# sithu/ByzantineRandomizedConsensus

Hardware: AMD Instinct MI355X
Metric: decided consensus instances/sec (node) at n=64,f=21 (higher is better)
Workload: dtype u32

## Files before the change

byzantinerandomizedconsensus_amd/csrc/brc_step.h:

```cpp
#pragma once
#include "brc_internal.h"
#include "schedule.h"

namespace brc {

constexpr uint32_t NOKEY = 0xFFFFFFFFu;
constexpr uint32_t TB_S = 1, TB_E = 2, TB_R = 4, TB_SH = 12, TB_KEY = (1u << TB_SH) - 1u;
constexpr uint32_t KL_SND_SH = 15, KL_DT_SH = 21, KL_RESTR = 1u << 25;

template <int NPAD> struct MaskOf { using type = uint64_t; };
template <> struct MaskOf<4> { using type = uint8_t; };
template <> struct MaskOf<8> { using type = uint8_t; };
template <> struct MaskOf<16> { using type = uint16_t; };
template <> struct MaskOf<32> { using type = uint32_t; };

template <typename T> __device__ __forceinline__ uint32_t popc(T x) { return (uint32_t)__popcll((uint64_t)x); }


__device__ __forceinline__ uint32_t dpp_row_or(uint32_t x) {
    x |= (uint32_t)__builtin_amdgcn_mov_dpp((int)x, 0xB1, 0xF, 0xF, true);
    x |= (uint32_t)__builtin_amdgcn_mov_dpp((int)x, 0x4E, 0xF, 0xF, true);
    x |= (uint32_t)__builtin_amdgcn_mov_dpp((int)x, 0x141, 0xF, 0xF, true);
    x |= (uint32_t)__builtin_amdgcn_mov_dpp((int)x, 0x140, 0xF, 0xF, true);
    return x;
// ... 66 lines not shown
        x = (x | (x >> 3)) & 0x0303030303030303ull; x = (x | (x >> 6)) & 0x000F000F000F000Full;
        x = (x | (x >> 12)) & 0x000000FF000000FFull;
        return (x | (x >> 24)) & 0xFFFFull;
    }
    if (G == 8) {
        x = (x | (x >> 7)) & 0x0003000300030003ull; x = (x | (x >> 14)) & 0x0000000F0000000Full;
        return (x | (x >> 28)) & 0xFFull;
    }
    if (G == 16) {
        x = (x | (x >> 15)) & 0x0000000300000003ull;
        return (x | (x >> 30)) & 0xFull;
    }
    return (x | (x >> 31)) & 0x3ull;
}

template <int I> struct IC { static constexpr int value = I; };
template <int N> struct Unrolled {
    template <typename F> __device__ __forceinline__ static void run(F&& f) {
        Unrolled<N - 1>::run(f);
        f(IC<N - 1>{});
    }
};
template <> struct Unrolled<0> {
    template <typename F> __device__ __forceinline__ static void run(F&&) {}
};

__device__ __forceinline__ uint32_t uni32(uint32_t x) { return (uint32_t)__builtin_amdgcn_readfirstlane((int)x); }
__device__ __forceinline__ uint64_t uni64(uint64_t x) {
    return (uint64_t)uni32((uint32_t)x) | ((uint64_t)uni32((uint32_t)(x >> 32)) << 32);
}
__device__ __forceinline__ uint64_t readlane64(uint64_t x, int l) {
    return (uint64_t)(uint32_t)__builtin_amdgcn_readlane((int)(uint32_t)x, l) |
           ((uint64_t)(uint32_t)__builtin_amdgcn_readlane((int)(uint32_t)(x >> 32), l) << 32);
}

template <typename T> using gptr_t = __attribute__((address_space(1))) T*;
template <typename T> __device__ __forceinline__ gptr_t<T> gp(T* p) { return (gptr_t<T>)p; }

__device__ __forceinline__ InjDev load_inj(const InjDev* p) {
    const gptr_t<const uint64_t> q = gp((const uint64_t*)p);
    const uint64_t w[3] = {q[0], q[1], q[2]};
    InjDev r;
    __builtin_memcpy(&r, w, 24);
    r.dst_hi[0] = r.dst_hi[1] = r.dst_hi[2] = 0;
    return r;
}

__device__ __forceinline__ uint32_t m_s1(uint64_t m) { return (uint32_t)(m & 0xFFFF); }
__device__ __forceinline__ uint32_t m_tsend(uint64_t m) { return (uint32_t)((m >> 16) & 0xFFFF); }
__device__ __forceinline__ uint32_t m_tquiet(uint64_t m) { return (uint32_t)((m >> 32) & 0xFFFF); }
__device__ __forceinline__ uint32_t m_sender(uint64_t m) { return (uint32_t)((m >> 48) & 0xFF); }
__device__ __forceinline__ uint32_t m_value(uint64_t m) { return (uint32_t)((m >> 56) & 0x7F); }
constexpr uint64_t M_RESTRICTED = 1ull << 63;
__device__ __forceinline__ uint64_t m_pack(uint32_t s1, uint32_t tsend, uint32_t tquiet, uint32_t sender, uint32_t value) {
    return (uint64_t)(s1 & 0xFFFF) | ((uint64_t)(tsend & 0xFFFF) << 16) | ((uint64_t)(tquiet & 0xFFFF) << 32) |
           ((uint64_t)(sender & 0xFF) << 48) | ((uint64_t)(value & 0xFF) << 56);
}
__device__ __forceinline__ uint64_t m_with_tquiet(uint64_t m, uint32_t q) {
    return (m & ~(0xFFFFull << 32)) | ((uint64_t)(q & 0xFFFF) << 32);
}

__device__ __forceinline__ void brb_cell_update(uint32_t& fl, uint32_t& ec, uint32_t& rc, bool s_arr,
                                                uint32_t ea, uint32_t ra, uint32_t T_echo, uint32_t T_amp,
                                                uint32_t T_del, bool& echo_send, bool& ready_send, bool& deliver) {
    const bool open = !(fl & F_DEL);
    const bool es_st = open && s_arr && !(fl & F_EEX);
    echo_send = es_st && !(fl & F_ES);
    fl |= es_st ? (F_EEX | F_ES) : 0u;
    const bool e_on = open && ea != 0;
    const uint32_t checked = (fl & F_EEX) ? ea : ea - 1u;
    fl |= e_on ? F_EEX : 0u;
    ec += e_on ? ea : 0u;
    const bool r1s = e_on && checked != 0 && ec >= T_echo && !(fl & F_REX);
    const bool r1 = r1s && !(fl & F_RS);
    fl |= r1s ? (F_REX | F_RS) : 0u;
    const bool r_on = open && ra != 0;
    const bool rex = (fl & F_REX) != 0;
    const uint32_t lo = rex ? rc + 1u : 2u, hi = rex ? rc + ra : ra;
    fl |= r_on ? F_REX : 0u;
    rc += r_on ? ra : 0u;
    const bool any = r_on && hi >= lo;
    const uint32_t alo = max(lo, T_amp), ahi = min(hi, T_del - 1u);
    const bool r2 = any & !(fl & F_EEX) & (alo <= ahi) & !(fl & F_RS);
    fl |= r2 ? F_RS : 0u;
    deliver = any && hi >= T_del;
    fl |= deliver ? F_DEL : 0u;
    ready_send = r1 || r2;
}

__device__ __forceinline__ void brb_cell_update_spec(uint32_t& fl, uint32_t& ec, uint32_t& rc, bool s_arr,
                                                     uint32_t ea, uint32_t ra, uint32_t T_echo, uint32_t T_amp,
                                                     uint32_t T_del, bool& echo_send, bool& ready_send, bool& deliver) {
    const bool open = !(fl & F_DEL);
    echo_send = open && s_arr && !(fl & F_ES);
    fl |= echo_send ? F_ES : 0u;
    ec += open ? ea : 0u;
    rc += open ? ra : 0u;
    ready_send = open && !(fl & F_RS) && (ec >= T_echo || rc >= T_amp);
    fl |= ready_send ? F_RS : 0u;
    deliver = open && rc >= T_del;
    fl |= deliver ? F_DEL : 0u;
}

__device__ __forceinline__ void brb_cell_update_beb(uint32_t& fl, bool s_arr, bool& echo_send, bool& ready_send,
                                                    bool& deliver) {
    deliver = s_arr && !(fl & F_DEL);
// ... 34 lines not shown
    const uint64_t w = r.lo ^ ((r.lo ^ r.hi) & (0ull - (uint64_t)((s >> 3) & 1u)));
    return (uint32_t)(w >> (8u * (s & 7u))) & 0xFFu;
}
__device__ __forceinline__ Ring16 ring_put(Ring16 r, uint32_t tl, uint32_t t, uint32_t c) {
    if (tl == NEVER || t - tl >= 16u) {
        r.lo = r.hi = 0;
    } else {
        for (uint32_t s = tl + 1u; s != t + 1u; ++s) {
            const uint64_t m = ~(0xFFull << (8u * (s & 7u)));
            if (s & 8u) r.hi &= m; else r.lo &= m;
        }
    }
    const uint64_t v = (uint64_t)min(c, RING_MAX) << (8u * (t & 7u)), m = ~(0xFFull << (8u * (t & 7u)));
    if (t & 8u) r.hi = (r.hi & m) | v; else r.lo = (r.lo & m) | v;
    return r;
}

#ifndef BRC_NL_MSTORE
#define BRC_NL_MSTORE 1
#endif
#ifndef BRC_LPK
#define BRC_LPK 1
#endif
#ifndef BRC_MIN_WAVES
#define BRC_MIN_WAVES 4
#endif
#ifndef BRC_MIN_WAVES_LEAN
#define BRC_MIN_WAVES_LEAN 4
#endif
#ifndef BRC_MIN_WAVES_LEAN_SPEC
#define BRC_MIN_WAVES_LEAN_SPEC 4
#endif
#ifndef BRC_SPEC_MULTI
#define BRC_SPEC_MULTI 1
#endif
#ifndef BRC_PERKEY_CNT
#define BRC_PERKEY_CNT 1
#endif
#ifndef BRC_BRANCHLESS
#define BRC_BRANCHLESS 0
#endif
#ifndef BRC_NOEARLY
#define BRC_NOEARLY 0
#endif
#ifndef BRC_LCHUNK_SPEC
#define BRC_LCHUNK_SPEC 4
#endif
#ifndef BRC_DACC
#define BRC_DACC 1
#endif
#ifndef BRC_OOBST
#define BRC_OOBST 1
#endif
#ifndef BRC_PK
#define BRC_PK 1
#endif
constexpr int TCLS = BRC_TYPED_ER ? 5 : 4;
constexpr int tcls_tb(int c) { return c == 1 ? 2 : c == 2 ? 4 : c == 3 ? 1 : c == 4 ? 6 : -1; }

typedef uint16_t u16x2 __attribute__((ext_vector_type(2)));
__device__ __forceinline__ uint32_t pk_add(uint32_t a, uint32_t b) {
    return __builtin_bit_cast(uint32_t, __builtin_bit_cast(u16x2, a) + __builtin_bit_cast(u16x2, b));
}
__device__ __forceinline__ uint32_t pk_sub(uint32_t a, uint32_t b) {
    return __builtin_bit_cast(uint32_t, __builtin_bit_cast(u16x2, a) - __builtin_bit_cast(u16x2, b));
}
__device__ __forceinline__ uint32_t pk_min(uint32_t a, uint32_t b) {
    return __builtin_bit_cast(uint32_t, __builtin_elementwise_min(__builtin_bit_cast(u16x2, a), __builtin_bit_cast(u16x2, b)));
}
__device__ __forceinline__ uint32_t pk_max(uint32_t a, uint32_t b) {
    return __builtin_bit_cast(uint32_t, __builtin_elementwise_max(__builtin_bit_cast(u16x2, a), __builtin_bit_cast(u16x2, b)));
}
__device__ __forceinline__ uint32_t pk_ge(uint32_t a, uint32_t b) { return (~pk_sub(a, b) >> 15) & 0x10001u; }
__device__ __forceinline__ uint32_t pk2(uint32_t x) { return x | (x << 16); }

#ifdef BRC_STAMPS
#define BRC_NSTAMPS 24
__device__ unsigned long long brc_stamps[BRC_NSTAMPS];
#endif
template <int NPAD, int MODE> constexpr bool lean_kernel() { return NPAD == 64 && MODE != KMODE_CONN && MODE != KMODE_XREF; }

#ifndef BRC_MIN_WAVES_EV
#define BRC_MIN_WAVES_EV 2
#endif
template <int NPAD, int DM, bool EV, int MODE, int NLR>
__global__ __launch_bounds__(64 * WPB, (EV ? BRC_MIN_WAVES_EV
                                           : lean_kernel<NPAD, MODE>() ? (MODE == BRC_MODE_SPEC ? BRC_MIN_WAVES_LEAN_SPEC
                                                                                              : BRC_MIN_WAVES_LEAN)
                                                                       : BRC_MIN_WAVES))
void brc_step(const Params* __restrict__ pp) {
    const Params& P = *pp;
    constexpr bool SPEC = MODE == BRC_MODE_SPEC, BEB = MODE == BRC_MODE_BEB, CONN = MODE == KMODE_CONN;
    constexpr bool LEAN = lean_kernel<NPAD, MODE>();
    constexpr bool TYPED = typed_list(LEAN, EV, MODE);
    static_assert(NLR == 0 || (LEAN && NLR == 2), "register delay masks: lean kernels, two delays");
    constexpr uint32_t CW = CONN ? 5 : 1;
    using T = typename MaskOf<NPAD>::type;
    constexpr uint32_t RS = ring_steps(DM);
    constexpr int IPW = 64 / NPAD;
    constexpr uint32_t AT = act_types(LEAN, IPW);
    constexpr bool PSEG = BRC_PSEG && !LEAN && IPW > 1;
    constexpr uint32_t NVAL = value_ids(!LEAN), VB = LEAN ? 2u : 3u, VMASK = NVAL - 1u;
    constexpr uint32_t VREP = LEAN ? 0x55u : 0x249249u;
    extern __shared__ __attribute__((aligned(16))) uint64_t smem[];

    const int wid = (int)uni32(threadIdx.x / 64), lane = threadIdx.x % 64;
    const uint64_t item = (uint64_t)blockIdx.x * WPB + wid;
    if (item >= P.nitems) return;
    const uint32_t n = P.n, NK = P.NK, Q = P.Q, NV = P.NV, D = P.D, nkw = P.nkw;
    const uint32_t T_echo = P.T_echo, T_amp = P.T_amp, T_del = P.T_del;
    const uint32_t qsh = (uint32_t)__ffs(Q) - 1u, Qm = Q - 1u, ksh = qsh + (uint32_t)__ffs(NV) - 1u;
    const uint32_t nL = NLR ? 0u : P.nL;
    const uint32_t h_words = cons_words(SPEC, (uint32_t)sizeof(T), Q, NV, NVAL);
    const bool seen_on = NV > 1;
    const uint32_t l_words = (nL * 64 * (uint32_t)sizeof(T) + 7) / 8;
    uint64_t* s_meta = smem + (size_t)wid * (lds_bytes_per_wave(NPAD, NK, nkw, nL, SPEC, Q, NV, RS, LEAN, TYPED) / 8);
    uint64_t* s_act = s_meta + IPW * NK;
    constexpr bool DBG = LEAN && SPEC;
    const uint32_t dbw = DBG ? 0u : 64u * nkw;
    uint64_t* s_dbits = s_act + RS * nkw * AT;
    T* s_hm = (T*)(s_dbits + dbw);
    T* s_seen = s_hm;
    uint32_t* s_cnt = (uint32_t*)(s_seen + (seen_on ? Q * 64 : 0u));
    T* s_L = (T*)(s_dbits + dbw + h_words);
    uint16_t* s_gen = (uint16_t*)(s_dbits + dbw + h_words + l_words);
    uint16_t* s_klist = s_gen + (LEAN ? 0u : ((IPW * NK + 3) & ~3u));
    const uint32_t KLS = NK + 2 * KPAD;
    constexpr bool KL32 = LEAN && (!SPEC || BRC_KL32_SPEC);
    uint32_t* s_klist32 = (uint32_t*)s_klist;
    uint64_t* s_injc = (uint64_t*)(s_klist + ((KLS * (PSEG ? IPW : 1u) + 3) & ~3u));

    const int seg = lane / NPAD, d = lane % NPAD, segbase = seg * NPAD;
    const uint64_t inst = item * IPW + seg;
    const bool iex = inst < P.instances;
    const uint64_t g = P.inst_offset + inst;
    const uint64_t all64 = (n >= 64) ? ~0ull : ((1ull << n) - 1);
    const T allm = (T)all64;
    const uint64_t segbits = (NPAD == 64) ? ~0ull : (((1ull << NPAD) - 1) << segbase);
    const uint32_t mbase = seg * NK;

    ItemState its = P.items[item];
    uint32_t t = LEAN ? uni32(its.t) : its.t, inj_pos = LEAN ? uni32(its.inj_pos) : its.inj_pos;
    uint32_t ep = LEAN ? uni32(its.epoch) : 0u;
    const uint32_t inj_off = gp(P.inj_off)[item], inj_cnt = gp(P.inj_cnt)[item];
    uint32_t injc_base = 0x80000000u;
    auto inj_at = [&](uint32_t pos) -> InjDev {
        if constexpr (LEAN) {
// ... 86 lines not shown
    const uint32_t maxout = hibit(outset);
    const uint32_t dset = wave_or_all(outset);
    uint64_t dlist = 0;
    uint32_t ndl = 0;
    for (uint32_t ds = dset; ds; ds &= ds - 1) dlist |= (uint64_t)(__ffs(ds) - 1) << (4 * ndl++);
    dlist = uni64(dlist); ndl = uni32(ndl);
    T RL0 = 0, RL1 = 0;
    constexpr bool LPK = NLR == 0 && BRC_LPK && sizeof(T) * DM <= 8;
    uint64_t Lpk = 0;
    uint32_t dly0 = 0, dly1 = 0;
    uint64_t OV0 = 0, OV1 = 0;
    if constexpr (NLR != 0) {
        if (ndl > 2) ovf = true;
        dly0 = ndl > 0 ? (uint32_t)(dlist & 15) + 1u : 0u;
        dly1 = ndl > 1 ? (uint32_t)((dlist >> 4) & 15) + 1u : 0u;
#pragma unroll
        for (int i = 0; i < DM; ++i) {
            if ((uint32_t)i + 1 == dly0) RL0 = L[i];
            if ((uint32_t)i + 1 == dly1) RL1 = L[i];
        }
        if (ndl > 0) OV0 = uni64(readlane64(outv, (int)dly0 - 1));
        if (ndl > 1) OV1 = uni64(readlane64(outv, (int)dly1 - 1));
    } else {
        uint32_t j = 0;
#pragma unroll
        for (int i = 0; i < DM; ++i)
            if ((dset >> i) & 1) {
                if (j < nL) s_L[j * 64 + lane] = L[i];
                if constexpr (LPK) Lpk |= (uint64_t)L[i] << ((j * 8 * sizeof(T)) & 63);
                ++j;
            }
        if (j > nL) ovf = true;
    }
    const uint64_t mk_ov = (lane & 1) ? OV1 : OV0;
    auto Lmask = [&](uint32_t j) -> T {
        if constexpr (NLR != 0) return j == 0 ? RL0 : RL1;
        else if constexpr (LPK) return (T)(Lpk >> ((j * 8 * sizeof(T)) & 63));
        else return s_L[j * 64 + lane];
    };
    const gptr_t<uint64_t> mycells = gp(P.cells) + item * (uint64_t)(NK + 1) * CW * 64 + lane;
    const gptr_t<uint64_t> gdbits = gp(P.dbits) + item * (uint64_t)nkw * 64 + lane;
    const __amdgpu_buffer_rsrc_t crs =
        __builtin_amdgcn_make_buffer_rsrc((void*)((uint32_t*)P.cells + item * (uint64_t)(NK + 1) * 64), (short)0,
                                          (int)((NK + 1) * 256u), 0x00020000);
    const uint32_t lv4 = (uint32_t)lane * 4u;
    auto cld = [&](uint32_t k) -> uint32_t { return __builtin_amdgcn_raw_buffer_load_b32(crs, lv4, k * 256u, 0); };
    auto cst = [&](uint32_t k, uint32_t v) { __builtin_amdgcn_raw_buffer_store_b32(v, crs, lv4, k * 256u, 0); };
    auto cst_if = [&](uint32_t k, uint32_t v, bool wr) {
        if constexpr (BRC_OOBST) __builtin_amdgcn_raw_buffer_store_b32(v, crs, wr ? lv4 : 0x80000000u, k * 256u, 0);
        else if (wr) cst(k, v);
    };
    uint32_t clr = 0;
    auto flush_clears = [&]() {
        if constexpr (LEAN) {
            for (uint64_t b = __ballot(clr != 0); b; b &= b - 1) {
                const int L = __ffsll((unsigned long long)b) - 1;
                for (uint32_t cm = uni32((uint32_t)__builtin_amdgcn_readlane((int)clr, L)); cm; cm &= cm - 1) {
                    const uint32_t k = ((uint32_t)L * NV) * Q + (uint32_t)__ffs(cm) - 1u;
                    cst(k, C32_FRESH);
                }
            }
            clr = 0;
        }
    };
    auto rebase = [&]() {
        if constexpr (LEAN) {
            const uint32_t nep = t - C32_KEEP, delta = nep - ep;
            for (uint32_t k = 0; k < NK; ++k) {
                if (m_s1(uni64(s_meta[k])) == 0) continue;
                const uint32_t c = cld(k);
                uint32_t oE = (c >> C32_OE_SH) & 127u, oR = c >> C32_OR_SH;
                if (oE < C32_OLD) oE = oE >= delta ? oE - delta : C32_OLD;
                if (oR < C32_OLD) oR = oR >= delta ? oR - delta : C32_OLD;
                cst(k, (c & ((1u << C32_OE_SH) - 1u)) | (oE << C32_OE_SH) | (oR << C32_OR_SH));
            }
            ep = nep;
        }
    };

    uint64_t c0 = 0, c1 = 0;
    const size_t li = item * 64 + lane;
    const bool cons_lane = honest && P.protocol == BRC_PROTO_CONSENSUS;
    if (cons_lane) { c0 = gp(P.cons0)[li]; c1 = gp(P.cons1)[li]; }
    if constexpr (SPEC) {
        const T* gseen = (const T*)P.hmask;
        const uint32_t* gcnt = (const uint32_t*)((const char*)P.hmask + (seen_on ? P.nitems * Q * 64 * sizeof(T) : 0));
        for (uint32_t q = 0; q < Q; ++q) {
            if (seen_on) s_seen[q * 64 + lane] = cons_lane ? gp(gseen)[(item * Q + q) * 64 + lane] : (T)0;
            s_cnt[q * 64 + lane] = cons_lane ? gp(gcnt)[(item * Q + q) * 64 + lane] : 0u;
        }
    } else {
        for (uint32_t v = 0; v < NVAL; ++v)
            s_hm[v * 64 + lane] = cons_lane ? gp((const T*)P.hmask)[(item * NVAL + v) * 64 + lane] : (T)0;
    }
    uint32_t round = c0 & 0xFFFF, phase = (c0 >> 16) & 0xF, nvals = (c0 >> 20) & 0xF;
    uint32_t order = (c0 >> 24) & 0xFFFFFF, vcount = (c0 >> 48) & 0xFFFF;
    uint32_t dcount = c1 & 0xFFFF, frnd = (c1 >> 16) & 0xFFFF, ft = (c1 >> 32) & 0xFFFF;
    uint32_t fval = (c1 >> 48) & 0xFF, lval = (c1 >> 56) & 0xFF;

    uint32_t xs_n = LEAN ? 0u : uni32(gp(P.xsn)[item]);
    auto xs_ld = [&](uint32_t i) -> uint64_t { return uni64(gp(P.xsend)[item * (uint64_t)(3 * XSEND_MAX) + i]); };

    uint32_t st_msgs = 0, st_arr = 0, st_cells = 0, st_del = 0, st_loads = 0, st_smax = 0;
    uint32_t st_bcast = 0;
    uint32_t nk_lean = 0, nk_skip = 0;

    auto log_ev = [&](uint32_t kind, uint32_t node, uint32_t type, uint32_t a, uint32_t b, uint32_t v) {
        if (EV) {
            const unsigned long long i = atomicAdd(P.event_count, 1ull);
            if (i < P.event_cap) {
                brc_event e;
                e.instance = inst; e.t = t; e.kind = (uint8_t)kind; e.node = (uint8_t)node;
                e.type = (uint8_t)type; e.value = (uint8_t)v; e.a = a; e.b = b;
                P.events[i] = e;
            }
        }
    };
    auto mark_lane = [&](uint32_t k, uint32_t ds, uint32_t ty) {
        while (ds) {
            const uint32_t i = __ffs(ds) - 1; ds &= ds - 1;
            const uint32_t row = (t + i + 1) & (RS - 1);
            if (!LEAN || ty != BRC_SEND)
                atomicOr((unsigned long long*)&s_act[(row * AT + (LEAN ? ty - BRC_ECHO : PSEG ? (uint32_t)seg : 0u)) * nkw + (k >> 6)],
                         1ull << (k & 63));
            lane_rows |= 1u << row;
        }
    };
    auto ring_busy = [&](uint32_t k) -> bool {
        const uint32_t kw = k >> 6, cur = t & (RS - 1);
        uint64_t acc = 0;
#pragma unroll 1
        for (uint32_t r = 0; r < RS; ++r)
            if (r != cur) acc |= s_act[(r * AT + 0) * nkw + kw] | s_act[(r * AT + 1) * nkw + kw];
        return (acc >> (k & 63)) & 1ull;
    };
    auto send_key_now = [&](uint32_t s, uint32_t v) {
        const uint32_t k = (d * NV) * Q + (s & Qm);
        const uint64_t m = s_meta[mbase + k];
        if ((m_s1(m) != 0 && (t < m_tquiet(m) || (LEAN && ring_busy(k)))) || s >= P.s_limit) { ovf = true; return; }
        if (!LEAN) s_gen[mbase + k] = (uint16_t)(((s_gen[mbase + k] & GEN_MASK) + 1) & GEN_MASK);
        if (LEAN) clr |= 1u << (s & Qm);
        s_meta[mbase + k] = m_pack(s + 1, t, t + maxout, d, v);
        mark_lane(k, outset, BRC_SEND);
        q_until = max(q_until, t + maxout);
        st_msgs += n;
        st_smax = max(st_smax, s);
        log_ev(BRC_EV_SEND, d, BRC_SEND, d * NV, s, v);
    };
    bool defer_sends = false;
    uint32_t sq_s = 0, sq_n = 0;
    SendQ<VB> sq_v;
    sq_v.clear();
    auto send_key = [&](uint32_t s, uint32_t v) {
        if (defer_sends) {
            if (sq_n == 0) sq_s = s;
            if (s == sq_s + sq_n && sq_n < SENDQ_MAX) { sq_v.put(sq_n, v & VMASK); ++sq_n; }
            else ovf = true;
            return;
        }
        send_key_now(s, v);
    };
    auto flush_sends = [&]() {
        for (uint32_t i = 0; i < sq_n; ++i) send_key_now(sq_s + i, sq_v.get(i) & VMASK);
        sq_n = 0; sq_v.clear();
    };
    auto get_max_val = [&](uint32_t bound2) -> uint32_t {
        for (uint32_t i = 0; i < nvals; ++i) {
            const uint32_t v = (order >> (VB * i)) & VMASK;
            if (2 * popc(s_hm[v * 64 + lane]) > bound2) return v;
        }
        return 0;
    };
    auto cons_reset = [&]() {
        vcount = 0; nvals = 0; order = 0;
        for (uint32_t v = 0; v < NVAL; ++v) s_hm[v * 64 + lane] = 0;
    };
    auto cons_after = [&]() {
        if (vcount >= P.T_cnt && phase == 1) {
            const uint32_t prop = get_max_val(P.bound_p1);
            phase = 2; cons_reset();
            send_key(2 * (round - 1) + 1, prop);
        }
        if (vcount >= P.T_cnt && phase == 2) {
            const uint32_t dec = get_max_val(P.bound_p2);
            ++dcount;
            if (dcount == 1) { frnd = round; ft = t; fval = dec; }
            lval = dec;
            log_ev(BRC_EV_DECIDE, d, 0, round, dec, dec);
            ++round; phase = 1; cons_reset();
            send_key(2 * (round - 1), dec);
        }
    };
    auto cons_deliver_vh = [&](uint32_t v, uint32_t host) {
        const uint32_t x = order ^ (v * VREP);
        const uint32_t valid = (1u << (VB * nvals)) - 1u;
// ... 83 lines not shown
                if (c > RING_MAX) {
                    badinj = true;
                } else {
                    sent = true;
                    ring = ring_put(ring, tl, t, c);
                    mycells[ri] = ring.lo;
                    mycells[ri + 64] = ring.hi;
                    log_ev((wv & bit) ? BRC_EV_COPY : BRC_EV_SEND, d, r.type, (k >> qsh), r.s, m_value(m));
                    wv = ((wv | bit) & ~(0xFFFFull << sh)) | ((uint64_t)t << sh);
                    mycells[(size_t)k * (CW * 64)] = wv;
                    st_msgs += n;
                }
            } else if (!(wv & bit)) {
                sent = true;
                wv |= bit;
                wv = (wv & ~(0xFFFFull << sh)) | ((uint64_t)t << sh);
                mycells[(size_t)k * (CW * 64)] = wv;
                st_msgs += n;
                log_ev(BRC_EV_SEND, d, r.type, (k >> qsh), r.s, m_value(m));
            }
        }
        return sent;
    };
    auto msg_marks = [&](const InjDev& r, bool mine, bool sent) {
        const uint32_t k = r.slot;
        const uint32_t os = wave_or(sent ? outset : 0u);
        if (os) {
            if (lane == 0) mark_lane(k, os, r.type);
            const uint32_t myq = seg_max<NPAD>(sent ? t + maxout : 0u);
            if (mine && myq) {
                if (d == 0) {
                    const uint64_t m = s_meta[mbase + k];
                    if (myq > m_tquiet(m)) s_meta[mbase + k] = m_with_tquiet(m, myq);
                }
                q_until = max(q_until, myq);
            }
        }
    };

    auto send_rec = [&](const InjDev& r, const uint32_t os) -> bool {
        const bool is_send = r.kind == BRC_INJ_SEND;
        const uint32_t k = r.slot;
        bool fresh = false;
        if (d == 0) {
            uint64_t m = s_meta[mbase + k];
            uint32_t gen = LEAN ? 0u : s_gen[mbase + k] & GEN_MASK;
            const bool declared = m_s1(m) == r.s + 1u && m_tsend(m) == NEVER && is_send;
            if ((!declared && m_s1(m) != 0 && (t < m_tquiet(m) || (LEAN && ring_busy(k)))) || r.s >= P.s_limit) {
                ovf = true;
            } else {
                uint32_t tq = m_tquiet(m);
                if (!declared) { gen = (gen + 1) & GEN_MASK; tq = t + 1; fresh = true; }
                if (is_send) tq = max(tq, t + hibit(os));
                m = m_pack(r.s + 1, is_send ? t : NEVER, tq, r.node, (uint32_t)(uint8_t)r.value);
                s_meta[mbase + k] = m;
                const bool restricted = is_send && (r.dst & all64) != all64;
                if (!LEAN) s_gen[mbase + k] = (uint16_t)(gen | (restricted ? GEN16_RESTRICTED : 0u));
                if (LEAN && restricted) s_meta[mbase + k] = m | M_RESTRICTED;
                st_smax = max(st_smax, (uint32_t)r.s);
                if (is_send) {
                    gp(P.kdst)[inst * NK + k] = r.dst;
                    mark_lane(k, os, BRC_SEND);
                    st_msgs += __popcll(r.dst & all64);
                    log_ev(BRC_EV_SEND, r.node, BRC_SEND, (k >> qsh), r.s, (uint32_t)(uint8_t)r.value);
                }
            }
        }
        return fresh;
    };
    auto send_delay_set = [&](const InjDev& r, const bool mine) -> uint32_t {
        uint32_t myset = 0;
        if (r.kind == BRC_INJ_SEND && mine && honest && ((r.dst >> d) & 1ull)) {
            uint32_t j = 0;
            for (uint32_t ds = dset; ds; ds &= ds - 1, ++j)
                if ((Lmask(j) >> r.node) & 1) myset = 1u << (__ffs(ds) - 1);
        }
        return myset;
    };

    auto do_actions = [&]() -> bool {
        bool mine_any = false;
        const bool running = status == BRC_RUNNING;
        if (its.initialized == 0 && t == 0) {
            if (P.protocol == BRC_PROTO_CONSENSUS && P.proposals != BRC_PROPOSALS_NONE && honest && running) {
                const uint32_t v = (P.proposals == BRC_PROPOSALS_PHILOX) ? proposal_id(P.seed, g, d)
                                                                         : (uint32_t)gp(P.prop)[inst * n + d];
                round = 1; phase = 1;
                send_key(0, v & (SPEC ? 3u : VMASK));
                if constexpr (SPEC) spec_advance();
            }
            flush_clears();
        }
        while (inj_pos < inj_cnt) {
            const InjDev r = inj_at(inj_pos);
            if (r.t != t) break;
            ++inj_pos;
            const bool mine = running && seg == (int)r.seg;
            mine_any |= mine;
            if (r.kind == BRC_INJ_PROPOSE) {
                if (mine && honest && d == r.node) {
                    round = 1; phase = 1; send_key(0, (uint32_t)r.value & (SPEC ? 3u : VMASK));
                    if constexpr (SPEC) spec_advance();
                }
            } else if (r.kind == BRC_INJ_DELIVER) {
                if constexpr (!SPEC) {
                    if (mine && honest && d == r.node) cons_deliver_vh((uint32_t)r.value & VMASK, r.slot);
                }
            } else if (!LEAN && IPW > 1 && (r.kind == BRC_INJ_SEND || r.kind == BRC_INJ_KEY) && !(r.type & 2u)) {
                const uint32_t p0 = inj_pos - 1;
                uint32_t p1 = inj_pos;
                while (p1 < inj_cnt && p1 - injc_base < INJ_CACHE) {
                    const InjDev q = inj_at(p1);
                    if (q.t != t || (q.kind != BRC_INJ_SEND && q.kind != BRC_INJ_KEY) || (q.type & 2u)) break;
                    ++p1;
                }
                inj_pos = p1;
                uint32_t myrecs = 0;
                for (uint32_t p = p0; p < p1; ++p)
                    if (seg == (int)inj_at(p).seg) myrecs |= 1u << (p - p0);
                while (__any(myrecs != 0)) {
                    InjDev q = r;
                    const bool has = myrecs != 0;
                    if (has) {
                        const uint32_t i = (uint32_t)__ffs(myrecs) - 1u;
                        myrecs &= myrecs - 1;
                        q = inj_at(p0 + i);
                    }
                    const bool mq = has && running;
                    mine_any |= mq;
                    const uint32_t os = seg_or<NPAD, uint32_t>(send_delay_set(q, mq));
                    if (mq) {
                        send_rec(q, os);
                        q_until = max(q_until, t + hibit(os));
                    }
                }
            } else if (r.kind == BRC_INJ_SEND || r.kind == BRC_INJ_KEY) {
                const uint32_t os = wave_or(send_delay_set(r, mine));
                if (!LEAN && (r.type & 2u)) {
                    if (mine && d == 0) {
                        const uint32_t k = r.slot;
                        const uint64_t m = s_meta[mbase + k];
                        if (m_s1(m) != r.s + 1u || m_tsend(m) == NEVER) {
                            badinj = true;
                        } else {
                            if (t + hibit(os) > m_tquiet(m)) s_meta[mbase + k] = m_with_tquiet(m, t + hibit(os));
                            mark_lane(k, os, BRC_SEND);
                            st_msgs += __popcll(r.dst & all64);
                            if (!(r.type & 1u)) log_ev(BRC_EV_SEND, r.node, BRC_SEND, (k >> qsh), r.s, m_value(m));
                            else if (CONN) log_ev(BRC_EV_COPY, r.node, BRC_SEND, (k >> qsh), r.s, m_value(m));
                        }
                    }
                    if (mine) q_until = max(q_until, t + hibit(os));
                } else if (mine) {
                    const bool fresh = send_rec(r, os);
                    if constexpr (LEAN) {
                        if (__ballot(fresh)) cst(uni32((uint32_t)r.slot), C32_FRESH);
                    }
                    q_until = max(q_until, t + hibit(os));
                }
            } else if (r.kind == BRC_INJ_MSG) {
                if constexpr (!LEAN) {
                  if (r.restricted) {
                    uint32_t myset = 0;
                    if (mine && honest && ((r.dst >> d) & 1ull)) {
                        uint32_t j = 0;
                        for (uint32_t ds = dset; ds; ds &= ds - 1, ++j)
                            if ((Lmask(j) >> r.node) & 1) myset = 1u << (__ffs(ds) - 1);
                    }
                    const uint32_t os = wave_or(myset);
                    if (mine && d == 0) {
                        const uint32_t k = r.slot;
                        const uint64_t m = s_meta[mbase + k];
                        if (m_s1(m) != r.s + 1u) {
                            badinj = true;
                        } else {
                            if (t + hibit(os) > m_tquiet(m)) s_meta[mbase + k] = m_with_tquiet(m, t + hibit(os));
                            mark_lane(k, os, r.type);
                            st_msgs += __popcll(r.dst & all64);
                            if (r.restricted & 2u) log_ev(BRC_EV_SEND, r.node, r.type, (k >> qsh), r.s, m_value(m));
                        }
                    }
                    if (mine) q_until = max(q_until, t + hibit(os));
                  } else {
                    const uint32_t p0 = inj_pos - 1;
                    uint32_t p1 = inj_pos;
                    while (p1 < inj_cnt && p1 - injc_base < INJ_CACHE) {
                        const InjDev q = inj_at(p1);
                        if (q.t != t || q.kind != BRC_INJ_MSG || q.restricted) break;
                        ++p1;
                    }
                    inj_pos = p1;
                    uint32_t myrecs = 0;
                    for (uint32_t p = p0; p < p1; ++p) {
                        const InjDev q = inj_at(p);
                        const bool mq = running && seg == (int)q.seg;
                        mine_any |= mq;
                        if (mq && d == q.node) myrecs |= 1u << (p - p0);
                    }
                    while (__any(myrecs != 0)) {
                        if (myrecs) {
                            const uint32_t i = (uint32_t)__ffs(myrecs) - 1u;
                            myrecs &= myrecs - 1;
                            const InjDev q = inj_at(p0 + i);
                            if (msg_cell(q) && outset) {
                                mark_lane(q.slot, outset, q.type);
                                const uint32_t myq = t + maxout;
                                q_until = max(q_until, myq);
                                unsigned long long* mp = (unsigned long long*)&s_meta[mbase + q.slot];
                                unsigned long long cur = *mp;
                                while (m_tquiet(cur) < myq) {
                                    const unsigned long long prev = atomicCAS(mp, cur, (unsigned long long)m_with_tquiet(cur, myq));
                                    if (prev == cur) break;
                                    cur = prev;
                                }
                            }
                        }
                    }
                  }
                } else {
                    msg_marks(r, mine, (mine && d == r.node) ? msg_cell(r) : false);
                }
            }
            flush_clears();
        }
        its.initialized = 1;
        return mine_any;
    };

    __builtin_amdgcn_fence(__ATOMIC_SEQ_CST, "wavefront");
    if (its.initialized == 0 && t == 0) {
        do_actions();
        q_until = NPAD == 64 ? wave_max_all(q_until) : seg_max<NPAD>(q_until);
        any_rows |= wave_or_all(lane_rows);
        lane_rows = 0;
        __builtin_amdgcn_fence(__ATOMIC_SEQ_CST, "wavefront");
    }

#ifdef BRC_STAMPS
    uint64_t stamp_acc[8] = {0, 0, 0, 0, 0, 0, 0, 0};
    uint32_t kcount[16] = {0, 0, 0, 0, 0, 0, 0, 0, 0, 0, 0, 0, 0, 0, 0, 0};
    uint64_t stamp_prev = __builtin_amdgcn_s_memtime();
#define BRC_STAMP(i) do { const uint64_t _n = __builtin_amdgcn_s_memtime(); stamp_acc[i] += _n - stamp_prev; stamp_prev = _n; } while (0)
#define BRC_KCOUNT(i) (++kcount[i])
#define BRC_KCOUNT_N(i, n) (kcount[i] += (n))
#else
#define BRC_STAMP(i) do {} while (0)
#define BRC_KCOUNT(i) do {} while (0)
#define BRC_KCOUNT_N(i, n) do {} while (0)
#endif
    for (uint32_t it = 0; it < P.max_steps; ++it) {
        const bool running0 = status == BRC_RUNNING;
        if (!__any(running0)) break;
        const bool running = IPW == 1 || running0;
        const bool hon_run = honest && running, real_run = real && running;
        const uint32_t rot = (t + 1) & (RS - 1);
        const uint32_t rr = (rot ? ((any_rows >> rot) | (any_rows << (RS - rot))) : any_rows) &
                            (RS == 32 ? ~0u : ((1u << RS) - 1u));
        uint32_t next = rr ? t + (uint32_t)__ffs(rr) : 0xFFFFFFFFu;
        if (inj_pos < inj_cnt) next = min(next, inj_at(inj_pos).t);
        if (next == 0xFFFFFFFFu) { if (running) status = BRC_QUIESCENT; break; }
        if (next > P.step_cap) { if (running) status = BRC_STEPCAP; break; }
        const bool reenter = next == t;
        t = LEAN ? uni32(next) : next;
        const uint32_t tsl = reenter ? (t | 0x40000000u) : t;
        const uint32_t row = t & (RS - 1);
        if (LEAN && t - ep > C32_REBASE) rebase();

        const uint32_t cells0 = st_cells;
        uint64_t dacc = 0;
        uint32_t dcur = NOKEY, dwm = 0;
        auto flush_dacc = [&](uint32_t wk, uint64_t v) {
            if (TYPED && ((dwm >> wk) & 1u)) {
                if constexpr (DBG) gdbits[wk * 64] = gdbits[wk * 64] | v;
                else s_dbits[wk * 64 + lane] |= v;
            } else {
                if constexpr (DBG) gdbits[wk * 64] = v;
                else s_dbits[wk * 64 + lane] = v;
            }
            dwm |= 1u << wk;
        };
        uint32_t nkeys = 0, nks = 0;
        uint32_t sbase[TCLS + 1], scnt[TCLS];
        if constexpr (LEAN) {
            auto slot_entry = [&](const uint32_t w, uint32_t& ent, bool& restr) -> uint32_t {
                const uint64_t mE = uni64(s_act[(row * AT + 0) * nkw + w]), mR = uni64(s_act[(row * AT + 1) * nkw + w]);
                const uint64_t m = s_meta[w * 64 + lane];
                const uint32_t dt = tsl - m_tsend(m);
                bool sl;
                if constexpr (NLR != 0) {
                    const uint32_t snd = m_sender(m) & 63u;
                    sl = m_s1(m) != 0 && ((dt == dly0 && ((OV0 >> snd) & 1ull)) || (dt == dly1 && ((OV1 >> snd) & 1ull)));
                } else {
                    const uint32_t dt1 = dt - 1u;
                    const uint32_t os = (uint32_t)__shfl((int)outset, (int)m_sender(m));
                    sl = m_s1(m) != 0 && dt1 < 32u && ((os >> (dt1 & 31u)) & 1u);
                }
                const uint32_t tb = (sl ? TB_S : 0u) | ((uint32_t)(mE >> lane) & 1u) * TB_E | ((uint32_t)(mR >> lane) & 1u) * TB_R;
                restr = (m & M_RESTRICTED) != 0;
                if constexpr (KL32) {
                    const uint32_t sx = (tb & TB_S) ? (((m_sender(m) & 63u) << KL_SND_SH) | (((dt - 1u) & 15u) << KL_DT_SH) |
                                                       (restr ? KL_RESTR : 0u)) : 0u;
                    ent = (w * 64 + lane) | (tb << TB_SH) | sx;
                } else {
                    ent = (w * 64 + lane) | (tb << TB_SH);
                }
                return tb;
            };
            auto put_entry = [&](const uint32_t pos, const uint32_t ent) {
                if constexpr (KL32) s_klist32[pos] = ent;
                else s_klist[pos] = (uint16_t)ent;
            };
            if constexpr (TYPED) {
                auto slot_class = [&](const uint32_t tb, const bool restr) -> uint32_t {
                    return tb == TB_E ? 1u : tb == TB_R ? 2u : (tb == TB_S && !restr) ? 3u
                                                              : (BRC_TYPED_ER && tb == (TB_E | TB_R)) ? 4u : 0u;
                };
                constexpr uint32_t LCT = SPEC ? BRC_LCHUNK_SPEC : LCHUNK;
#pragma unroll
                for (int c = 0; c < TCLS; ++c) scnt[c] = 0;
                for (uint32_t w = 0; w < nkw; ++w) {
                    uint32_t ent;
                    bool restr;
                    const uint32_t tb = slot_entry(w, ent, restr), cl = slot_class(tb, restr);
#ifdef BRC_STAMPS
                    for (uint32_t v = 1; v < 8; ++v) BRC_KCOUNT_N(4 + v, (uint32_t)__popcll(__ballot(tb == v)));
#endif
                    Unrolled<TCLS>::run([&](auto ci) {
                        constexpr int c = decltype(ci)::value;
                        scnt[c] += (uint32_t)__popcll(__ballot(tb != 0 && cl == (uint32_t)c));
                    });
                }
                sbase[0] = 0;
#pragma unroll
                for (int c = 0; c < TCLS; ++c) sbase[c + 1] = sbase[c] + ((scnt[c] + LCT - 1u) & ~(LCT - 1u));
                uint32_t spos[TCLS];
#pragma unroll
                for (int c = 0; c < TCLS; ++c) spos[c] = sbase[c];
                for (uint32_t w = 0; w < nkw; ++w) {
                    uint32_t ent;
                    bool restr;
                    const uint32_t tb = slot_entry(w, ent, restr), cl = slot_class(tb, restr);
                    Unrolled<TCLS>::run([&](auto ci) {
                        constexpr int c = decltype(ci)::value;
                        const bool in = tb != 0 && cl == (uint32_t)c;
                        const uint64_t bits = __ballot(in);
                        const uint32_t below = __builtin_amdgcn_mbcnt_hi((uint32_t)(bits >> 32),
                                                                         __builtin_amdgcn_mbcnt_lo((uint32_t)bits, 0u));
                        if (in) put_entry(spos[c] + below, ent);
                        spos[c] += (uint32_t)__popcll(bits);
                    });
                }
                Unrolled<TCLS>::run([&](auto ci) {
                    constexpr int c = decltype(ci)::value;
                    if (spos[c] + lane < sbase[c + 1]) put_entry(spos[c] + lane, NK);
                    nk_lean += scnt[c];
                });
                nkeys = sbase[TCLS];
            } else {
            for (uint32_t w = 0; w < nkw; ++w) {
                uint32_t ent;
                bool restr;
                const uint32_t tb = slot_entry(w, ent, restr);
                const uint64_t bits = __ballot(tb != 0);
                const uint32_t below = __builtin_amdgcn_mbcnt_hi((uint32_t)(bits >> 32),
                                                                 __builtin_amdgcn_mbcnt_lo((uint32_t)bits, 0u));
#ifdef BRC_STAMPS
                for (uint32_t v = 1; v < 8; ++v) BRC_KCOUNT_N(4 + v, (uint32_t)__popcll(__ballot(tb == v)));
#endif
                if (tb != 0) put_entry(nkeys + below, ent);
                nkeys += (uint32_t)__popcll(bits);
            }
            }
        } else if constexpr (PSEG) {
            for (uint32_t w = 0; w < nkw; ++w) {
                const uint64_t bits = s_act[(row * AT + (uint32_t)seg) * nkw + w];
                for (uint32_t b0 = 0; b0 < 64; b0 += NPAD) {
                    const uint32_t b = b0 + (uint32_t)d;
                    if ((bits >> b) & 1ull)
                        s_klist[(uint32_t)seg * KLS + nks + (uint32_t)__popcll(bits & ((1ull << b) - 1ull))] = (uint16_t)(w * 64 + b);
                }
                nks += (uint32_t)__popcll(bits);
            }
            nkeys = wave_max_all(nks);
        } else {
            for (uint32_t w = 0; w < nkw; ++w) {
                const uint64_t bits = uni64(s_act[row * nkw + w]);
                const uint32_t below = __builtin_amdgcn_mbcnt_hi((uint32_t)(bits >> 32),
                                                                 __builtin_amdgcn_mbcnt_lo((uint32_t)bits, 0u));
                if ((bits >> lane) & 1) s_klist[nkeys + below] = (uint16_t)(w * 64 + lane);
                nkeys += (uint32_t)__popcll(bits);
            }
        }
        if (!PSEG && lane < 2 * KPAD) {
            if constexpr (KL32) s_klist32[nkeys + lane] = NK;
            else s_klist[nkeys + lane] = (uint16_t)NK;
        }
        if constexpr (LEAN && !TYPED) nk_lean += nkeys;
        (void)sbase; (void)scnt;
        __builtin_amdgcn_fence(__ATOMIC_SEQ_CST, "wavefront");
        BRC_STAMP(0);
        auto fetch = [&](uint32_t p, uint64_t (&ww)[CHUNK], uint32_t (&kk)[CHUNK]) {
            Unrolled<CHUNK>::run([&](auto ci) {
                constexpr int c = decltype(ci)::value;
// ... 730 lines not shown
                        for (int j = 1; j < 8; ++j) b = i == (uint32_t)j ? bv[j] : b;
                        cons_word((uint32_t)(wv >> (5 * i)) & 31u, b);
                    }
                }
            } else {
#pragma unroll 1
                for (uint32_t w = 0; w < nkw; ++w) {
                    const uint64_t bits = s_dbits[w * 64 + lane];
                    s_dbits[w * 64 + lane] = 0;
                    cons_word(w, bits);
                }
            }
            }
        }
        BRC_STAMP(2);
        defer_sends = false;
        flush_sends();
        flush_clears();
        __builtin_amdgcn_fence(__ATOMIC_SEQ_CST, "wavefront");
        BRC_STAMP(6);

        const bool inj_mine = do_actions();
        any_rows |= wave_or_all(lane_rows);
        lane_rows = 0;
        __builtin_amdgcn_fence(__ATOMIC_SEQ_CST, "wavefront");
        BRC_STAMP(3);

        q_until = NPAD == 64 ? wave_max_all(q_until) : seg_max<NPAD>(q_until);
        const uint64_t b_act = __ballot(st_cells != cells0 || inj_mine) & segbits;
        const uint64_t b_ovf = __ballot(ovf) & segbits;
        const uint64_t b_bad = __ballot(badinj) & segbits;
        const uint64_t b_und = __ballot(honest && dcount < P.round_cap) & segbits;
        uint32_t seg_pending = 0;
        if (__any(running && q_until <= t && inj_pos < inj_cnt))
            for (uint32_t p = inj_pos; p < inj_cnt; ++p) seg_pending |= 1u << inj_at(p).seg;
        if (running) {
            if (b_act) t_stop = t;
            if (b_bad) status = BRC_BADINJ;
            else if (b_ovf) status = BRC_OVERFLOW;
            else if (P.protocol == BRC_PROTO_CONSENSUS && P.round_cap > 0 && !b_und) status = BRC_DONE;
            else if (q_until <= t && !((seg_pending >> seg) & 1u)) status = BRC_QUIESCENT;
        }
        for (uint32_t i = lane; i < nkw * AT; i += 64) s_act[row * nkw * AT + i] = 0;
        any_rows &= ~(1u << row);
        __builtin_amdgcn_fence(__ATOMIC_SEQ_CST, "wavefront");
        BRC_STAMP(4);
    }

#ifdef BRC_STAMPS
    if (lane == 0) for (int i = 0; i < 8; ++i) atomicAdd(&brc_stamps[i], (unsigned long long)stamp_acc[i]);
    if (lane == 0) for (int i = 0; i < 16; ++i) atomicAdd(&brc_stamps[8 + i], (unsigned long long)kcount[i]);
#endif
#undef BRC_STAMP
    {
        const uint64_t mb = item * IPW * (uint64_t)NK;
        for (uint32_t i = lane; i < IPW * NK; i += 64) {
            if (item * IPW + i / NK < P.instances) {
                gp(P.meta)[mb + i] = s_meta[i] & ~M_RESTRICTED;
                gp(P.mgen)[mb + i] = LEAN ? ((s_meta[i] & M_RESTRICTED) ? GEN_RESTRICTED : 0u) : gen32(s_gen[i]);
            }
        }
        for (uint32_t i = lane; i < RS * nkw * AT; i += 64) gp(P.act)[item * RS * nkw * AT + i] = s_act[i];
    }
    if (lane == 0) {
        gp(P.actany)[item] = any_rows;
        ItemState o = {t, inj_pos, 1u, ep};
        P.items[item] = o;
    }
    if (honest && P.protocol == BRC_PROTO_CONSENSUS) {
        gp(P.cons0)[li] = cons0_pack(round, phase, nvals, order, vcount);
        gp(P.cons1)[li] = (uint64_t)(dcount & 0xFFFF) | ((uint64_t)(frnd & 0xFFFF) << 16) | ((uint64_t)(ft & 0xFFFF) << 32) |
                      ((uint64_t)(fval & 0xFF) << 48) | ((uint64_t)(lval & 0xFF) << 56);
        if constexpr (SPEC) {
            T* gseen = (T*)P.hmask;
            uint32_t* gcnt = (uint32_t*)((char*)P.hmask + (seen_on ? P.nitems * Q * 64 * sizeof(T) : 0));
            for (uint32_t q = 0; q < Q; ++q) {
                if (seen_on) gp(gseen)[(item * Q + q) * 64 + lane] = s_seen[q * 64 + lane];
                gp(gcnt)[(item * Q + q) * 64 + lane] = s_cnt[q * 64 + lane];
            }
        } else {
            for (uint32_t v = 0; v < NVAL; ++v) gp((T*)P.hmask)[(item * NVAL + v) * 64 + lane] = s_hm[v * 64 + lane];
        }
    }
    if (LEAN && lane != 0) { st_cells = 0; st_del = 0; st_bcast = 0; }
    if (LEAN && !honest) st_arr = 0;
    st_msgs += st_bcast * n;
    if (LEAN && real) st_loads += nk_lean - nk_skip;
    uint32_t sums[4] = {st_msgs, st_arr, st_cells, st_del};
#pragma unroll
    for (int q = 0; q < 4; ++q) {
#pragma unroll
        for (int o = NPAD / 2; o; o >>= 1) sums[q] += (uint32_t)__shfl_xor((int)sums[q], o);
    }
    if (iex && d == 0) {
        gptr_t<uint64_t> ip = (gptr_t<uint64_t>)&gp(P.inst)[inst];
        *ip = (*ip & 0xFFFF000000000000ull) | (uint64_t)(status & 0xFFFF) | ((uint64_t)(t_stop & 0xFFFF) << 16) |
              ((uint64_t)(q_until & 0xFFFF) << 32);
        gp(P.istats)[inst * 4 + 0] += sums[0];
        gp(P.istats)[inst * 4 + 1] += sums[1];
        gp(P.istats)[inst * 4 + 2] += sums[2];
        gp(P.istats)[inst * 4 + 3] += sums[3];
    }
    uint64_t w6[5] = {st_cells, st_arr, st_msgs, st_del, st_loads};
#pragma unroll
    for (int q = 0; q < 5; ++q) {
#pragma unroll
        for (int o = 32; o; o >>= 1) w6[q] += (uint64_t)__shfl_xor((unsigned long long)w6[q], o);
    }
    uint32_t smax = st_smax;
#pragma unroll
    for (int o = 32; o; o >>= 1) smax = max(smax, (uint32_t)__shfl_xor((int)smax, o));
// ... 53 lines not shown
```

Baseline: 8.146 million.

## Defer fresh-slot cell clears via meta flag and fast-path fresh sends

Adds an M_FRESH bit in slot metadata so that reinitialising a reused slot's cells is deferred, not done eagerly at send time (flush_clears and the per-send cst are disabled). Fresh unrestricted sends get their own class in the typed key list and are resolved directly: per-lane hit computation, a single cell store, and activation-mask updates. This skips the regular cell load/update path for them. Other paths lazily clear the flag on first touch (fresh_row, rebase skip, a final sweep before write-back). This removes redundant cell clears and cell loads for first-time deliveries, at the cost of extra ballots and serial per-slot loops and more complex state invariants.

```diff
diff --git a/byzantinerandomizedconsensus_amd/csrc/brc_step.h b/byzantinerandomizedconsensus_amd/csrc/brc_step.h
--- a/byzantinerandomizedconsensus_amd/csrc/brc_step.h
+++ b/byzantinerandomizedconsensus_amd/csrc/brc_step.h
@@ -142,6 +142,7 @@
 __device__ __forceinline__ uint32_t m_sender(uint64_t m) { return (uint32_t)((m >> 48) & 0xFF); }
 __device__ __forceinline__ uint32_t m_value(uint64_t m) { return (uint32_t)((m >> 56) & 0x7F); }
 constexpr uint64_t M_RESTRICTED = 1ull << 63;
+constexpr uint64_t M_FRESH = 1ull << 62;
 __device__ __forceinline__ uint64_t m_pack(uint32_t s1, uint32_t tsend, uint32_t tquiet, uint32_t sender, uint32_t value) {
     return (uint64_t)(s1 & 0xFFFF) | ((uint64_t)(tsend & 0xFFFF) << 16) | ((uint64_t)(tquiet & 0xFFFF) << 32) |
            ((uint64_t)(sender & 0xFF) << 48) | ((uint64_t)(value & 0xFF) << 56);
@@ -282,6 +283,9 @@
 #ifndef BRC_OOBST
 #define BRC_OOBST 1
 #endif
+#ifndef BRC_FRESH_SEND
+#define BRC_FRESH_SEND 1
+#endif
 #ifndef BRC_PK
 #define BRC_PK 1
 #endif
@@ -323,6 +327,7 @@
     constexpr bool SPEC = MODE == BRC_MODE_SPEC, BEB = MODE == BRC_MODE_BEB, CONN = MODE == KMODE_CONN;
     constexpr bool LEAN = lean_kernel<NPAD, MODE>();
     constexpr bool TYPED = typed_list(LEAN, EV, MODE);
+    constexpr bool FRESH = BRC_FRESH_SEND && TYPED;
     static_assert(NLR == 0 || (LEAN && NLR == 2), "register delay masks: lean kernels, two delays");
     constexpr uint32_t CW = CONN ? 5 : 1;
     using T = typename MaskOf<NPAD>::type;
@@ -515,7 +520,7 @@
     };
     uint32_t clr = 0;
     auto flush_clears = [&]() {
-        if constexpr (LEAN) {
+        if constexpr (LEAN && !FRESH) {
             for (uint64_t b = __ballot(clr != 0); b; b &= b - 1) {
                 const int L = __ffsll((unsigned long long)b) - 1;
                 for (uint32_t cm = uni32((uint32_t)__builtin_amdgcn_readlane((int)clr, L)); cm; cm &= cm - 1) {
@@ -526,11 +531,36 @@
             clr = 0;
         }
     };
+    auto fresh_row = [&](const uint32_t k) {
+        if constexpr (FRESH) {
+            if (k < NK) {
+                const uint64_t m = uni64(s_meta[k]);
+                if (m & M_FRESH) {
+                    cst(k, C32_FRESH);
+                    if (lane == 0) s_meta[k] = m & ~M_FRESH;
+                }
+            }
+        }
+    };
+    auto fresh_rows_all = [&]() {
+        if constexpr (FRESH) {
+            for (uint32_t w = 0; w < nkw; ++w) {
+                const uint64_t m = s_meta[w * 64 + lane];
+                uint64_t fb = __ballot((m & M_FRESH) != 0);
+                if (fb) {
+                    if (m & M_FRESH) s_meta[w * 64 + lane] = m & ~M_FRESH;
+                    for (; fb; fb &= fb - 1) cst(w * 64 + (uint32_t)__ffsll((unsigned long long)fb) - 1u, C32_FRESH);
+                }
+            }
+        }
+    };
     auto rebase = [&]() {
         if constexpr (LEAN) {
             const uint32_t nep = t - C32_KEEP, delta = nep - ep;
             for (uint32_t k = 0; k < NK; ++k) {
-                if (m_s1(uni64(s_meta[k])) == 0) continue;
+                const uint64_t mk = uni64(s_meta[k]);
+                if (m_s1(mk) == 0) continue;
+                if (FRESH && (mk & M_FRESH)) continue;
                 const uint32_t c = cld(k);
                 uint32_t oE = (c >> C32_OE_SH) & 127u, oR = c >> C32_OR_SH;
                 if (oE < C32_OLD) oE = oE >= delta ? oE - delta : C32_OLD;
@@ -602,8 +632,8 @@
         const uint64_t m = s_meta[mbase + k];
         if ((m_s1(m) != 0 && (t < m_tquiet(m) || (LEAN && ring_busy(k)))) || s >= P.s_limit) { ovf = true; return; }
         if (!LEAN) s_gen[mbase + k] = (uint16_t)(((s_gen[mbase + k] & GEN_MASK) + 1) & GEN_MASK);
-        if (LEAN) clr |= 1u << (s & Qm);
-        s_meta[mbase + k] = m_pack(s + 1, t, t + maxout, d, v);
+        if (LEAN && !FRESH) clr |= 1u << (s & Qm);
+        s_meta[mbase + k] = m_pack(s + 1, t, t + maxout, d, v) | (FRESH ? M_FRESH : 0ull);
         mark_lane(k, outset, BRC_SEND);
         q_until = max(q_until, t + maxout);
         st_msgs += n;
@@ -793,7 +823,8 @@
                 uint32_t tq = m_tquiet(m);
                 if (!declared) { gen = (gen + 1) & GEN_MASK; tq = t + 1; fresh = true; }
                 if (is_send) tq = max(tq, t + hibit(os));
-                m = m_pack(r.s + 1, is_send ? t : NEVER, tq, r.node, (uint32_t)(uint8_t)r.value);
+                const uint64_t mf = FRESH ? (fresh ? M_FRESH : m & M_FRESH) : 0ull;
+                m = m_pack(r.s + 1, is_send ? t : NEVER, tq, r.node, (uint32_t)(uint8_t)r.value) | mf;
                 s_meta[mbase + k] = m;
                 const bool restricted = is_send && (r.dst & all64) != all64;
                 if (!LEAN) s_gen[mbase + k] = (uint16_t)(gen | (restricted ? GEN16_RESTRICTED : 0u));
@@ -894,7 +925,7 @@
                     if (mine) q_until = max(q_until, t + hibit(os));
                 } else if (mine) {
                     const bool fresh = send_rec(r, os);
-                    if constexpr (LEAN) {
+                    if constexpr (LEAN && !FRESH) {
                         if (__ballot(fresh)) cst(uni32((uint32_t)r.slot), C32_FRESH);
                     }
                     q_until = max(q_until, t + hibit(os));
@@ -959,6 +990,7 @@
                     }
                   }
                 } else {
+                    fresh_row(uni32((uint32_t)r.slot));
                     msg_marks(r, mine, (mine && d == r.node) ? msg_cell(r) : false);
                 }
             }
@@ -1023,9 +1055,11 @@
         uint32_t nkeys = 0, nks = 0;
         uint32_t sbase[TCLS + 1], scnt[TCLS];
         if constexpr (LEAN) {
+            uint64_t se_m = 0;
             auto slot_entry = [&](const uint32_t w, uint32_t& ent, bool& restr) -> uint32_t {
                 const uint64_t mE = uni64(s_act[(row * AT + 0) * nkw + w]), mR = uni64(s_act[(row * AT + 1) * nkw + w]);
                 const uint64_t m = s_meta[w * 64 + lane];
+                se_m = m;
                 const uint32_t dt = tsl - m_tsend(m);
                 bool sl;
                 if constexpr (NLR != 0) {
@@ -1053,6 +1087,7 @@
             };
             if constexpr (TYPED) {
                 auto slot_class = [&](const uint32_t tb, const bool restr) -> uint32_t {
+                    if (FRESH && tb == TB_S && !restr && (se_m & M_FRESH)) return (uint32_t)TCLS;
                     return tb == TB_E ? 1u : tb == TB_R ? 2u : (tb == TB_S && !restr) ? 3u
                                                               : (BRC_TYPED_ER && tb == (TB_E | TB_R)) ? 4u : 0u;
                 };
@@ -1090,6 +1125,47 @@
                         if (in) put_entry(spos[c] + below, ent);
                         spos[c] += (uint32_t)__popcll(bits);
                     });
+                    if constexpr (FRESH) {
+                        const bool fr = tb != 0 && (se_m & M_FRESH) != 0;
+                        const uint64_t fall = __ballot(fr);
+                        if (fall) {
+                            uint64_t fs = __ballot(fr && cl == (uint32_t)TCLS);
+                            if (fr) s_meta[w * 64 + lane] = se_m & ~M_FRESH;
+                            nk_lean += (uint32_t)__popcll(fs);
+                            for (uint64_t b = fall & ~fs; b; b &= b - 1)
+                                cst(w * 64 + (uint32_t)__ffsll((unsigned long long)b) - 1u, C32_FRESH);
+                            const uint32_t hitw = (SPEC ? F_ES : (F_EEX | F_ES)) | ((t - ep) << C32_OE_SH) | (C32_NEVER << C32_OR_SH);
+                            for (; fs; fs &= fs - 1) {
+                                const int sl = __ffsll((unsigned long long)fs) - 1;
+                                const uint64_t mk = readlane64(se_m, sl);
+                                const uint32_t snd = m_sender(mk) & 63u, dt = tsl - m_tsend(mk);
+                                bool hit;
+                                if constexpr (NLR != 0) {
+                                    hit = (((RL0 >> snd) & 1) != 0) == (dt == dly0);
+                                } else {
+                                    const uint32_t sj = popc(dset & ((1u << ((dt - 1u) & 31)) - 1u));
+                                    hit = (s_L[sj * 64 + lane] >> snd) & 1;
+                                }
+                                const uint64_t hm = __ballot(hit) & hon_mask;
+                                cst(w * 64 + (uint32_t)sl, lane_in(hm) ? hitw : C32_FRESH);
+                                st_cells += popc(hm);
+                                st_bcast += popc(hm);
+                                st_arr += lane_in(hm) ? 1u : 0u;
+                                if constexpr (NLR != 0) {
+                                    const uint32_t mrow = ((t + ((lane & 1) ? dly1 : dly0)) & (RS - 1)) * AT * nkw;
+                                    if (lane < 2 && (hm & mk_ov) != 0)
+                                        atomicOr((unsigned long long*)&s_act[mrow + w], 1ull << sl);
+                                } else {
+                                    for (uint32_t ds = dset; ds; ds &= ds - 1) {
+                                        const uint32_t j = (uint32_t)__ffs(ds) - 1;
+                                        const uint32_t r = (t + j + 1u) & (RS - 1);
+                                        if ((hm & readlane64(outv, (int)j)) != 0 && lane == 0)
+                                            atomicOr((unsigned long long*)&s_act[(r * AT + 0) * nkw + w], 1ull << sl);
+                                    }
+                                }
+                            }
+                        }
+                    }
                 }
                 Unrolled<TCLS>::run([&](auto ci) {
                     constexpr int c = decltype(ci)::value;
@@ -1926,11 +2002,12 @@
     if (lane == 0) for (int i = 0; i < 16; ++i) atomicAdd(&brc_stamps[8 + i], (unsigned long long)kcount[i]);
 #endif
 #undef BRC_STAMP
+    fresh_rows_all();
     {
         const uint64_t mb = item * IPW * (uint64_t)NK;
         for (uint32_t i = lane; i < IPW * NK; i += 64) {
             if (item * IPW + i / NK < P.instances) {
-                gp(P.meta)[mb + i] = s_meta[i] & ~M_RESTRICTED;
+                gp(P.meta)[mb + i] = s_meta[i] & ~(M_RESTRICTED | (FRESH ? M_FRESH : 0ull));
                 gp(P.mgen)[mb + i] = LEAN ? ((s_meta[i] & M_RESTRICTED) ? GEN_RESTRICTED : 0u) : gen32(s_gen[i]);
             }
         }
```

After: 8.994 million, median of 6. +10.4%, better.
